# filevich/freeimpala

Measured on AMD Instinct MI355X. Metric: learner env-steps/sec (T×B/step) at T=100 B=4096, 1/2/4/8 MI355X, higher is better.
Workload: dtype bf16; 1 GPU; config#3 Atari-shaped conv policy 84x84x4, bf16 MFMA GEMMs + fp32 V-trace; T=100, B_per_gpu=4096, A=18, global_batch=4096, seq_len=100, parallelism=dp1, optimizer=adam, policy=atari

## Files before the change

freeimpala_amd/build_info.py:

```python
from __future__ import annotations

import glob
import hashlib
import os

ROOT = os.path.dirname(os.path.dirname(os.path.abspath(__file__)))


def source_files():
    files = sorted(glob.glob(os.path.join(ROOT, "freeimpala_amd", "csrc", "*")))
    files = [f for f in files if os.path.basename(f) != "farmer.hip"]
    files += [os.path.join(ROOT, p) for p in ("include/fi_learner.h", "Makefile")]
    return [f for f in files if os.path.isfile(f)]


def source_hash() -> str:
    h = hashlib.sha256()
    for f in source_files():
        h.update(os.path.relpath(f, ROOT).encode() + b"\0")
        with open(f, "rb") as fh:
            h.update(fh.read())
        h.update(b"\0")
    return h.hexdigest()[:16]


KERNEL_ENV = ("FI_FR_GRID", "FI_KEEP_DA1", "FI_BWD_UNFUSED", "FI_FWD_UNFUSED",
              "FI_A1_NHWC", "FI_ATARI_GENERIC")


def rocm_version() -> str:
    for p in ("/opt/rocm/.info/version", "/opt/rocm/.info/version-dev"):
        try:
            with open(p) as fh:
                return fh.read().strip()
        except OSError:
            pass
    return "unknown"


def runtime_key() -> dict:
    return {"env": {k: os.environ[k] for k in KERNEL_ENV if k in os.environ}, "rocm": rocm_version()}

# ... 11 lines not shown
```

freeimpala_amd/csrc/atari.h:

```cpp
#pragma once

#include <hip/hip_runtime.h>
#include <stdint.h>

#include <vector>

namespace fi {

constexpr int kC1Segs = 8;

struct KernelTagger {
    virtual void begin(const char* name) = 0;
    virtual void end() = 0;
    virtual ~KernelTagger() {}
};
struct TagScope {
    KernelTagger* t;
    TagScope(KernelTagger* t_, const char* name) : t(t_) {
        if (t) t->begin(name);
    }
    ~TagScope() {
        if (t) t->end();
    }
};
// ... 1 lines not shown
struct GradReadyHook {
    virtual int ready(size_t off, size_t n) = 0;
    virtual ~GradReadyHook() {}
};

struct AtariNet {
    static constexpr size_t kFrameBytes = 84 * 84 * 4;
    int B = 0, T = 0, A = 0, N = 0;
    void* impl = nullptr;
};

size_t atari_param_count(int A);
void atari_init_params(int A, uint64_t seed, std::vector<float>& p);
AtariNet* atari_create(int B, int T, int A);
void atari_destroy(AtariNet* n);
int atari_sync_weights(AtariNet* n, const float* params, hipStream_t s);
int atari_forward(AtariNet* n, const uint8_t* frames, float* logits, float* values, hipStream_t s,
                  KernelTagger* tg = nullptr);
int atari_backward(AtariNet* n, const uint8_t* frames, const float* dlogits, const float* dvalue,
                   float* grads, hipStream_t s, KernelTagger* tg = nullptr, GradReadyHook* gr = nullptr);
bool atari_tensor(AtariNet* n, const char* name, void** p, size_t* bytes);

}
```

freeimpala_amd/csrc/atari.hip:

```cpp
#include <algorithm>
#include <cstdlib>
#include <vector>

#include "atari.h"
#include "fi_common.h"
#include "kernels.h"

namespace fi {

typedef __bf16 bf16x8 __attribute__((ext_vector_type(8)));
typedef __bf16 bf16x4 __attribute__((ext_vector_type(4)));
typedef float f32x16 __attribute__((ext_vector_type(16)));
typedef unsigned int u32x4 __attribute__((ext_vector_type(4)));

namespace geo {
constexpr int C1K = 256, C1O = 32;
constexpr int C2K = 512, C2O = 64;
constexpr int C3K = 576, C3O = 64;
constexpr int FCK = 3136, FCO = 512;
constexpr int HP = 32;
constexpr int P1 = 400, P2 = 81, P3 = 49;
}

struct Offsets {
// ... 538 lines not shown
                              __bf16* dh, int R, int TB, float* fcb_slab, hipStream_t s) {
    FI_TRY(heads_dispatch(O, [&](auto o) {
        hipLaunchKernelGGL(heads_dgrad_valu<decltype(o)::value>, dim3(kHeadsDgradGrid), dim3(256), 0, s, dlog,
                           dval, wh, h, dh, R, TB, fcb_slab);
        return FI_OK;
    }));
    FI_HIP_CHECK(hipGetLastError());
    return FI_OK;
}

struct WeightsBf16 {
    __bf16 *c1T, *c2T, *c3T, *fcT, *hT;
    __bf16 *c2D, *c3D, *fcB;
};

__global__ void weights_bf16_kernel(const float* __restrict__ p, Offsets o, int A, WeightsBf16 w) {
    const int O = A + 1;
    const size_t n1 = 32 * 256, n2 = 64 * 512, n3 = 64 * 576, nf = (size_t)512 * 3136,
                 nh = 32 * 512, n2d = 4 * 32 * 256, n3d = 64 * 576, nfb = nf;
    const size_t total = n1 + n2 + n3 + nf + nh + n2d + n3d + nfb;
    for (size_t t = blockIdx.x * (size_t)blockDim.x + threadIdx.x; t < total;
         t += (size_t)gridDim.x * blockDim.x) {
        size_t i = t;
        if (i < n1) { const int co = i / 256, k = i % 256; w.c1T[i] = (__bf16)p[o.c1w + (size_t)k * 32 + co]; continue; }
        i -= n1;
        if (i < n2) { const int co = i / 512, k = i % 512; w.c2T[i] = (__bf16)p[o.c2w + (size_t)k * 64 + co]; continue; }
        i -= n2;
        if (i < n3) { const int co = i / 576, k = i % 576; w.c3T[i] = (__bf16)p[o.c3w + (size_t)k * 64 + co]; continue; }
        i -= n3;
        if (i < nf) { const size_t j = i / 3136, k = i % 3136; w.fcT[i] = (__bf16)p[o.fcw + k * 512 + j]; continue; }
        i -= nf;
        if (i < nh) { const int oo = i / 512, j = i % 512; w.hT[i] = (__bf16)(oo < O ? p[o.hw + (size_t)j * O + oo] : 0.f); continue; }
        i -= nh;
        if (i < n2d) {
            const int cls = i / (32 * 256), r = i % (32 * 256), ci = r / 256, k = r % 256;
// ... 18 lines not shown
    Offsets off{18};
    WeightsBf16 wb{};
    __bf16 *a1 = nullptr, *a2 = nullptr, *a3 = nullptr, *h = nullptr;
    __bf16 *da1 = nullptr, *da2 = nullptr, *da3 = nullptr, *dh = nullptr;
    float* slab = nullptr;
    size_t slab_floats = 0;
    const float* params = nullptr;
    std::vector<void*> allocs;
    int cs2 = 0, cs3 = 0;
    bool fr = true;
    bool fuse12 = true;
    bool fuse21 = true;
    bool keep_da1 = false;
    bool a1_planar = true;
    int fr_grid = 256;
};

int conv1_fwd_fr_launch(const uint8_t* frames, const __bf16* w1t, const float* bias, __bf16* a1,
                        int nframes, int grid, hipStream_t s);
int conv2_fwd_fr_launch(const __bf16* a1, const __bf16* w2t, const float* bias, __bf16* a2, int nframes,
                        int grid, hipStream_t s);
int conv3_fwd_fr_launch(const __bf16* a2, const __bf16* w3t, const float* bias, __bf16* a3, int nframes,
                        int grid, hipStream_t s);
int conv12_fwd_fr_launch(const uint8_t* frames, const __bf16* w1t, const float* b1, const __bf16* w2t,
                         const float* b2, __bf16* a1, __bf16* a2, int nframes, int grid, hipStream_t s,
                         int a1_planar);
int conv1_wgrad_fr_launch(const uint8_t* frames, const __bf16* da1, float* slab, float* cs_slab,
                          int nframes, int grid, hipStream_t s);
int conv21_bwd_fr_launch(const __bf16* a1, const __bf16* da2, const __bf16* w2d, const uint8_t* frames,
                         __bf16* da1_out, float* slab2, float* cs2, float* slab1, float* cs1, int nframes,
// ... 36 lines not shown
    I->a1_planar = I->fr && I->fuse12 && I->fuse21 && std::getenv("FI_A1_NHWC") == nullptr;
    if (const char* g = std::getenv("FI_FR_GRID")) I->fr_grid = std::max(1, std::min(256, std::atoi(g)));
    I->cs2 = (int)(((N * 100) + GBM - 1) / GBM * GBM);
    I->cs3 = (int)(((N * 81) + GBM - 1) / GBM * GBM);
    bool ok = dmalloc(I, &I->a1, N * 400 * 32) && dmalloc(I, &I->a2, N * 81 * 64) &&
              dmalloc(I, &I->a3, N * 3136) && dmalloc(I, &I->h, N * 512) &&
              dmalloc(I, &I->da1, N * 400 * 32) && dmalloc(I, &I->da2, N * 81 * 64) &&
              dmalloc(I, &I->da3, N * 3136) && dmalloc(I, &I->dh, N * 512) &&
              dmalloc(I, &I->wb.c1T, 32 * 256) && dmalloc(I, &I->wb.c2T, 64 * 512) &&
              dmalloc(I, &I->wb.c3T, 64 * 576) && dmalloc(I, &I->wb.fcT, (size_t)512 * 3136) &&
              dmalloc(I, &I->wb.hT, 32 * 512) && dmalloc(I, &I->wb.c2D, 4 * 32 * 256) &&
              dmalloc(I, &I->wb.c3D, 64 * 576) && dmalloc(I, &I->wb.fcB, (size_t)3136 * 512);
    const size_t s_fc = (size_t)SPL_FC * 3136 * 512, s_c3 = (size_t)SPL_C3 * 576 * 64,
                 s_c2 = (size_t)SPL_C2 * (512 * 64 + kC1Segs * 256 * 32), s_c1 = (size_t)SPL_C1 * 256 * 32,
                 s_h = (size_t)kHeadsGrid * 512 * 19;
    I->slab_floats = std::max(std::max(s_fc, s_c3), std::max(std::max(s_c2, s_c1), s_h)) + 1024 * 512;
    ok = ok && dmalloc(I, &I->slab, I->slab_floats);
    if (!ok) {
        set_error("atari: hipMalloc failed for activations");
        atari_destroy(n);
        return nullptr;
    }
    hipStream_t s0;
    if (hipStreamCreate(&s0) != hipSuccess) {
        set_error("atari: hipStreamCreate failed");
        atari_destroy(n);
        return nullptr;
    }
    if (hipMemsetAsync(I->dh, 0, N * 512 * sizeof(__bf16), s0) != hipSuccess ||
        hipMemsetAsync(I->da3, 0, N * 3136 * sizeof(__bf16), s0) != hipSuccess ||
        hipMemsetAsync(I->da2, 0, N * 81 * 64 * sizeof(__bf16), s0) != hipSuccess ||
        hipMemsetAsync(I->da1, 0, N * 400 * 32 * sizeof(__bf16), s0) != hipSuccess || hipStreamSynchronize(s0) != hipSuccess) {
// ... 4 lines not shown
    }
    (void)hipStreamDestroy(s0);
    return n;
}

void atari_destroy(AtariNet* n) {
    if (!n) return;
    AtariImpl* I = impl(n);
    if (I) {
        for (void* p : I->allocs) (void)hipFree(p);
        delete I;
    }
    delete n;
}

int atari_sync_weights(AtariNet* n, const float* params, hipStream_t s) {
    AtariImpl* I = impl(n);
    I->params = params;
    hipLaunchKernelGGL(weights_bf16_kernel, dim3(2048), dim3(256), 0, s, params, I->off, I->A, I->wb);
    FI_HIP_CHECK(hipGetLastError());
    return FI_OK;
}

int atari_forward(AtariNet* n, const uint8_t* frames, float* logits, float* values, hipStream_t s,
                  KernelTagger* tg) {
    AtariImpl* I = impl(n);
    const int N = I->N;
    const float* p = I->params;
    const Offsets& o = I->off;
    using namespace geo;
    int rc;
    if (I->fr && I->fuse12) {
        TagScope ts(tg, "conv12_fwd");
        rc = conv12_fwd_fr_launch(frames, I->wb.c1T, p + o.c1b, I->wb.c2T, p + o.c2b, I->a1, I->a2, N,
                                  std::min(N, I->fr_grid), s, I->a1_planar);
    } else if (I->fr) {
// ... 24 lines not shown
                             EpiHeadsOut{logits, values, p + o.hb, I->A}, N, HP, FCO, s); }
    return rc;
}

int atari_backward(AtariNet* n, const uint8_t* frames, const float* dlogits, const float* dvalue,
                   float* grads, hipStream_t s, KernelTagger* tg, GradReadyHook* gr) {
    AtariImpl* I = impl(n);
    const int N = I->N, A = I->A, O = A + 1;
    const int Nb = I->TB;
    const Offsets& o = I->off;
    using namespace geo;
    float* slab = I->slab;
    float* cs = I->slab + I->slab_floats - 1024 * 512;
    int rc;
#define FI_A(tag, x) do { TagScope ts_(tg, tag); rc = (x); if (rc) return rc; } while (0)
    FI_A("heads_wgrad", heads_wgrad_launch(O, dlogits, dvalue, I->h, slab, cs, Nb, I->TB, s));
    FI_A("reduce_slabs", reduce_slabs(slab, kHeadsGrid, (size_t)FCO * O, grads + o.hw, s));
    FI_A("reduce_slabs", reduce_slabs(cs, kHeadsGrid, (size_t)O, grads + o.hb, s));
    FI_A("heads_dgrad", heads_dgrad_launch(O, dlogits, dvalue, I->params + o.hw, I->h, I->dh, Nb, I->TB, slab, s));
    FI_A("reduce_slabs", reduce_slabs(slab, kHeadsDgradGrid, (size_t)FCO, grads + o.fcb, s));
    FI_A("fc_wgrad", fc_wgrad_launch(I->a3, I->dh, slab, grads + o.fcw, Nb, s));
    if (gr && (rc = gr->ready(o.fcw, o.total - o.fcw))) return rc;
    FI_A("fc_dgrad", fc_dgrad_launch(I->dh, I->wb.fcB, I->da3, I->fr ? Nb : N, s));
    if (I->fr) {
        const int grid = std::min(N, I->fr_grid);
        FI_A("conv3_bwd", conv3_bwd_fr_launch(I->a2, I->da3, I->a3, I->wb.c3D, I->da2, slab, cs, cs + (size_t)3 * grid * C2O,
                                              Nb, grid, s));
        FI_A("reduce_slabs", reduce_slabs(slab, grid, (size_t)C3K * C3O, grads + o.c3w, s));
        FI_A("reduce_slabs", reduce_slabs(cs, grid, (size_t)C3O, grads + o.c3b, s));
        if (gr && (rc = gr->ready(o.c3w, o.fcw - o.c3w))) return rc;
    } else {
        FI_A("relu_mask", relu_mask_bf16(I->da3, I->a3, (size_t)N * FCK, s));
        FI_A("conv3_wgrad", (wgrad<128, 64, 2, 2>(ConvGather<9, 64, 3, 1, 7>{I->a2, N * P3}, RowsBf16{I->da3, N * P3, C3O},
                                   slab, cs, N * P3, C3K, C3O, SPL_C3, 1.f, s)));
        FI_A("reduce_slabs", reduce_slabs(slab, SPL_C3, (size_t)C3K * C3O, grads + o.c3w, s));
        FI_A("reduce_slabs", reduce_slabs(cs, SPL_C3, (size_t)C3O, grads + o.c3b, s));
        FI_A("conv3_dgrad", (gemm<128, 64, 2, 2>(DgradGather<9, 3, 1, 7, 64>{I->da3, N, I->cs3},
                                  ClassRows{I->wb.c3D, 64, C3K, I->cs3, (size_t)64 * C3K, nullptr},
                                  EpiDgrad<9, 1>{I->da2, I->a2, N, I->cs3, 64}, I->cs3, 64, C3K, s)));
        if (gr && (rc = gr->ready(o.c3w, o.fcw - o.c3w))) return rc;
    }
    if (I->fr && I->fuse21) {
        const int grid = std::min(N, I->fr_grid);
        float* slab1 = slab + (size_t)grid * C2K * C2O;
        float* cs1 = cs + (size_t)grid * C2O;
        FI_A("conv21_bwd", conv21_bwd_fr_launch(I->a1, I->da2, I->wb.c2D, frames, I->keep_da1 ? I->da1 : nullptr,
                                                slab, cs + (size_t)3 * grid * C2O, slab1, cs1, Nb, grid, s, I->a1_planar));
        FI_A("reduce_slabs", reduce_slabs(slab, grid, (size_t)C2K * C2O, grads + o.c2w, s));
        FI_A("reduce_slabs", reduce_slabs(cs + (size_t)3 * grid * C2O, 2 * grid, (size_t)C2O, grads + o.c2b, s));
        FI_A("reduce_slabs", reduce_slabs(slab1, grid * kC1Segs, (size_t)C1K * C1O, grads + o.c1w, s));
        FI_A("reduce_slabs", reduce_slabs(cs1, 4 * grid, (size_t)C1O, grads + o.c1b, s));
        if (gr && (rc = gr->ready(0, o.c3w))) return rc;
        return FI_OK;
    }
    if (I->fr) {
        const int grid = std::min(N, I->fr_grid);
        FI_A("conv2_bwd", conv2_bwd_fr_launch(I->a1, I->da2, I->wb.c2D, I->da1, slab, cs + (size_t)3 * grid * C2O, Nb,
                                              grid, s));
        FI_A("reduce_slabs", reduce_slabs(slab, grid, (size_t)C2K * C2O, grads + o.c2w, s));
        FI_A("reduce_slabs", reduce_slabs(cs + (size_t)3 * grid * C2O, 2 * grid, (size_t)C2O, grads + o.c2b, s));
    } else {
        FI_A("conv2_wgrad", (wgrad<128, 64, 2, 2>(ConvGather<20, 32, 4, 2, 9>{I->a1, N * P2}, RowsBf16{I->da2, N * P2, C2O},
                               slab, cs, N * P2, C2K, C2O, SPL_C2, 1.f, s)));
        FI_A("reduce_slabs", reduce_slabs(slab, SPL_C2, (size_t)C2K * C2O, grads + o.c2w, s));
        FI_A("reduce_slabs", reduce_slabs(cs, SPL_C2, (size_t)C2O, grads + o.c2b, s));
        FI_A("conv2_dgrad", (gemm<128, 32, 4, 1>(DgradGather<20, 4, 2, 9, 64>{I->da2, N, I->cs2},
                              ClassRows{I->wb.c2D, 32, 256, I->cs2, (size_t)32 * 256, nullptr},
                              EpiDgrad<20, 2>{I->da1, I->a1, N, I->cs2, 32}, 4 * I->cs2, 32, 256, s)));
    }
    if (I->fr) {
        const int grid = std::min(N, I->fr_grid);
        FI_A("conv1_wgrad", conv1_wgrad_fr_launch(frames, I->da1, slab, cs, Nb, grid, s));
        FI_A("reduce_slabs", reduce_slabs(slab, grid, (size_t)C1K * C1O, grads + o.c1w, s));
        FI_A("reduce_slabs", reduce_slabs(cs, grid, (size_t)C1O, grads + o.c1b, s));
    } else {
        FI_A("conv1_wgrad", (wgrad<128, 32, 4, 1>(Conv1Gather{frames, N * P1}, RowsBf16{I->da1, N * P1, C1O}, slab, cs,
                                   N * P1, C1K, C1O, SPL_C1, 1.0f / 255.0f, s)));
        FI_A("reduce_slabs", reduce_slabs(slab, SPL_C1, (size_t)C1K * C1O, grads + o.c1w, s));
        FI_A("reduce_slabs", reduce_slabs(cs, SPL_C1, (size_t)C1O, grads + o.c1b, s));
    }
    if (gr && (rc = gr->ready(0, o.c3w))) return rc;
#undef FI_A
    return FI_OK;
}

bool atari_tensor(AtariNet* n, const char* name, void** p, size_t* bytes) {
    AtariImpl* I = impl(n);
    const size_t N = I->N;
    struct E {
        const char* nm;
        void* p;
        size_t b;
    } t[] = {{"a1", I->a1, N * 400 * 32 * 2}, {"a2", I->a2, N * 81 * 64 * 2},
             {"a3", I->a3, N * 3136 * 2},     {"h", I->h, N * 512 * 2},
             {"da1", I->da1, N * 400 * 32 * 2}, {"da2", I->da2, N * 81 * 64 * 2},
             {"da3", I->da3, N * 3136 * 2},   {"dh", I->dh, N * 512 * 2}};
// ... 11 lines not shown
```

freeimpala_amd/csrc/fc_gemm.hip:

```cpp
#include <algorithm>

#include "fi_common.h"
#include "kernels.h"

namespace fi {
namespace fcg {

typedef __bf16 bf16x8 __attribute__((ext_vector_type(8)));
typedef __bf16 bf16x4 __attribute__((ext_vector_type(4)));
typedef float f32x4 __attribute__((ext_vector_type(4)));
typedef int i32x2 __attribute__((ext_vector_type(2)));
typedef int i32x4 __attribute__((ext_vector_type(4)));
typedef __attribute__((address_space(3))) bf16x4 lds_bf16x4;

constexpr int FCK = 3136, FCO = 512;

__device__ __forceinline__ void dma16(fi_i32x4 rsrc, uint32_t voff, uint32_t lds_base) {
    uint32_t keep;
    asm volatile(
        "s_nop 4\n\t"
        "s_mov_b32 %0, m0\n\t"
        "s_mov_b32 m0, %3\n\t"
        "s_nop 0\n\t"
        "buffer_load_dwordx4 %1, %2, 0 offen lds\n\t"
// ... 498 lines not shown
}

int fc_wgrad_splits(int rows) {
    return std::max(1, std::min(9, (rows + 255) / 256));
}

template <int BX, int BY, int WX, int WY, int BK, int NS>
static int fc_wgrad_impl(const __bf16* a3, const __bf16* dh, float* slab, float* dw, int rows, hipStream_t s,
                         int S) {
    FI_REQUIRE(rows > 0, "fc_wgrad: rows must be positive");
    const int rps = ((rows + S - 1) / S + BK - 1) / BK * BK;
    const int nblk = S * (FCO / BX) * (FCK / BY);
    hipLaunchKernelGGL((fc_tn_kernel<BX, BY, WX, WY, BK, NS>), dim3(nblk), dim3(512), 0, s, dh, FCO, a3, FCK, rows, rps,
                       slab);
    FI_HIP_CHECK(hipGetLastError());
    return reduce_slabs(slab, S, (size_t)FCK * FCO, dw, s);
}

int fc_fwd_launch(const __bf16* a3, const __bf16* wT, const float* bias, __bf16* h, int rows, hipStream_t s) {
    return fc_fwd_impl<FC_FW_CFG>(a3, wT, bias, h, rows, s);
}
int fc_dgrad_launch(const __bf16* dh, const __bf16* w, __bf16* da3, int rows, hipStream_t s) {
    return fc_dgrad_impl<FC_DG_CFG>(dh, w, da3, rows, s);
}
int fc_wgrad_launch(const __bf16* a3, const __bf16* dh, float* slab, float* dw, int rows, hipStream_t s) {
    return fc_wgrad_impl<FC_WG_CFG>(a3, dh, slab, dw, rows, s, fc_wgrad_splits(rows));
}

}
```

freeimpala_amd/csrc/kernels.h:

```cpp
#pragma once

#include <hip/hip_runtime.h>
#include <stdint.h>

#include "fi_learner.h"

namespace fi {

struct HeadsGrad {
    const float* dlog;
    const float* dval;
    int rows;
    int TB;
    int A;
};

size_t vtrace_workspace_bytes(int T, int B, int A);
int vtrace_launch(int variant, int T, int B, int A, const float* pi, const float* mu,
                  const int32_t* act, const float* rew, const float* disc, const float* val,
                  const fi_vtrace_hparams& hp, float* vs, float* adv, float* dlog, float* dval,
                  double* losses, void* ws, size_t ws_bytes, hipStream_t stream,
                  bool finalize = true, int* nblk_out = nullptr, int* bad = nullptr);
int vtrace_finalize_launch(void* ws, int nblk, double* losses, hipStream_t stream,
                           const int* bad = nullptr);
// ... 17 lines not shown
                        float* cs_slab, int grid, hipStream_t s);

int colsum_partial(const float* Y, int M, int N, int splits, float* slab, hipStream_t s);
int heads_colsum_partial(const HeadsGrad& g, int splits, float* slab, hipStream_t s);
int f32_gemm_nt(const float* X, int ldx, int M, int K, const float* W, const float* bias, int N,
                bool relu, float* Y, hipStream_t s);
int f32_gemm_nn_dgrad(const float* dY, int M, int N, const float* W, int K, const float* act, float* dX,
                      hipStream_t s);
int f32_gemm_tn_wgrad(const float* dY, int M, int N, const float* X, int ldx, int K, int splits, float* slab,
                      hipStream_t s);
int fc_fwd_launch(const __bf16* a3, const __bf16* wT, const float* bias, __bf16* h, int rows, hipStream_t s);
int fc_dgrad_launch(const __bf16* dh, const __bf16* w, __bf16* da3, int rows, hipStream_t s);
int fc_wgrad_splits(int rows);
int fc_wgrad_launch(const __bf16* a3, const __bf16* dh, float* slab, float* dw, int rows, hipStream_t s);
int reduce_slabs(float* slab, int splits, size_t count, float* out, hipStream_t s);
int grad_sqnorm(const float* g, size_t n, double* part, int nblk, double* out, hipStream_t s,
                const double* vt_part = nullptr, int vt_nblk = 0, double* vt_losses = nullptr,
                int* nonfinite = nullptr);
int optimizer_step(int opt, float* p, const float* g, float* m, float* v, size_t n, float lr,
                   float b1, float b2, float eps, double bc1, double bc2, const double* sqnorm,
                   float max_norm, hipStream_t s, int* skip = nullptr);
int to_bf16(const float* src, uint16_t* dst, size_t n, hipStream_t s);
int fill_hash_bf16(void* dst, size_t n, uint32_t seed, hipStream_t s);
int synth_launch(uint64_t seed, int T, int B, int B_glob, int b_off, int A, int D, float gamma,
                 float* obs, float* mu, int32_t* act, float* rew, float* disc, uint8_t* frames,
                 hipStream_t s);
int ingest_launch(const void* rec, int T, int B, int A, int D, size_t entry_bytes, float* obs,
                  float* mu, int32_t* act, float* rew, float* disc, hipStream_t s, int* bad = nullptr);
int ingest_atari_launch(const void* rec, int T, int B, int A, size_t entry_bytes, uint8_t* frames,
                        float* mu, int32_t* act, float* rew, float* disc, hipStream_t s,
                        int* bad = nullptr);
int ingest_atari_planes_launch(const void* rec, int T, int B, int A, size_t entry_bytes, uint8_t* frames,
                               float* mu, int32_t* act, float* rew, float* disc, hipStream_t s,
                               int* bad = nullptr);

}
// ... 1 lines not shown
```

freeimpala_amd/csrc/learner.cpp:

```cpp
#include <hip/hip_runtime.h>
#include <rccl/rccl.h>

#include <algorithm>
#include <chrono>
#include <cstdio>
#include <cstdlib>
#include <cmath>
#include <cstring>
#include <new>
#include <string>
#include <thread>
#include <vector>

#include "atari.h"
#include "fi_common.h"
#include "kernels.h"

namespace fi {

static thread_local std::string g_err;
void set_error(const std::string& msg) { g_err = msg; }
int fail(int code, const std::string& msg) {
    g_err = msg;
    return code;
// ... 539 lines not shown
    }
    mark(l, FI_PHASE_BACKWARD);
    BucketAllReduce bar(l);
    if (l->cfg.arch == FI_ARCH_MLP) FI_TRY(mlp_backward(l, &bar));
    else {
        LearnerTagger tg(l);
        FI_TRY(atari_backward(l->atari, l->frames, l->dlogits, l->dvalue, l->grads, l->stream,
                              l->profiling ? &tg : nullptr, &bar));
    }
    mark(l, FI_PHASE_ALLREDUCE);
    {
        Tag t(l, "allreduce_wait");
        FI_TRY(bar.join());
    }
    mark(l, FI_PHASE_OPTIMIZER);
    {
        Tag t(l, "grad_norm");
        FI_TRY(grad_sqnorm(l->grads, l->nparams, l->small + 8, kSqParts, l->small + 3, l->stream,
                           vtrace_partials(l->vt_ws), vt_nblk, l->small, l->bad + 1));
    }
    const int step = l->step_count + 1;
    const double bc1 = 1.0 - std::pow((double)l->cfg.beta1, step);
    const double bc2 = 1.0 - std::pow((double)l->cfg.beta2, step);
    {
        Tag t(l, "optimizer");
        FI_TRY(optimizer_step(l->cfg.optimizer, l->params, l->grads, l->opt_m, l->opt_v, l->nparams,
                              l->cfg.lr, l->cfg.beta1, l->cfg.beta2, l->cfg.eps, bc1, bc2,
                              l->small + 3, l->cfg.max_grad_norm, l->stream, l->bad));
    }
    if (l->atari) {
        Tag t(l, "weights_bf16");
        FI_TRY(atari_sync_weights(l->atari, l->params, l->stream));
    }
    mark(l, FI_PHASE_COUNT);
    if (out) FI_HIP_CHECK(hipEventRecord(l->ev_b, l->stream));
    l->step_count = step;
    l->version++;
    if (sync) {
        FI_HIP_CHECK(hipStreamSynchronize(l->stream));
        if (l->profiling) {
            for (int p = 0; p < FI_PHASE_COUNT; ++p) {
                float ms = 0.f;
                FI_HIP_CHECK(hipEventElapsedTime(&ms, l->ev[p], l->ev[p + 1]));
                l->phase_sum[p] += ms;
            }
            l->phase_steps++;
            collect_tags(l);
// ... 512 lines not shown
```

freeimpala_amd/csrc/misc.hip:

```cpp
#include <algorithm>

#include "fi_common.h"
#include "kernels.h"

namespace fi {

__device__ __forceinline__ float approx_normal(uint4 u) {
    const uint32_t s = (u.x >> 8) + (u.y >> 8) + (u.z >> 8) + (u.w >> 8);
    const float x = (float)((int32_t)s - (int32_t)(1u << 25));
    return x * 0x1.bb67aep-24f;
}

__global__ void synth_normal_kernel(uint64_t seed, uint32_t stream, int rows, int B, int B_glob,
                                    int b_off, int D, float* out) {
    const size_t n = (size_t)rows * B * D;
    for (size_t i = blockIdx.x * (size_t)blockDim.x + threadIdx.x; i < n;
         i += (size_t)gridDim.x * blockDim.x) {
        const size_t lrow = i / D;
        const int d = (int)(i - lrow * D);
        const int t = (int)(lrow / B), b = (int)(lrow - (size_t)t * B);
        const uint64_t row = (uint64_t)t * B_glob + (uint64_t)(b_off + b);
        out[i] = approx_normal(philox4(seed, row * D + d, stream));
    }
}
// ... 349 lines not shown
int reduce_slabs(float* slab, int splits, size_t count, float* out, hipStream_t s) {
    if (splits >= 4 * kSlabGroup && count < 32768) {
        const int groups = (splits + kSlabGroup - 1) / kSlabGroup;
        hipLaunchKernelGGL(reduce_slabs_stage1, dim3((unsigned)((count + 63) / 64), (unsigned)groups), dim3(64), 0, s,
                           slab, splits, count);
        hipLaunchKernelGGL(reduce_slabs_kernel, dim3((unsigned)((count + 63) / 64)), dim3(256), 0, s, slab, groups,
                           count, (size_t)kSlabGroup * count, out);
    } else {
        hipLaunchKernelGGL(reduce_slabs_kernel, dim3((unsigned)((count + 63) / 64)), dim3(256), 0, s, slab, splits,
                           count, count, out);
    }
    FI_HIP_CHECK(hipGetLastError());
    return FI_OK;
}

__global__ void sqnorm_part_kernel(const float* __restrict__ g, size_t n, double* part) {
    __shared__ double red[4];
    double s = 0.0;
    for (size_t i = blockIdx.x * (size_t)blockDim.x + threadIdx.x; i < n;
         i += (size_t)gridDim.x * blockDim.x)
        s += (double)g[i] * (double)g[i];
    s = wave_sum(s);
    if ((threadIdx.x & 63) == 0) red[threadIdx.x >> 6] = s;
    __syncthreads();
    if (threadIdx.x == 0) part[blockIdx.x] = (red[0] + red[1]) + (red[2] + red[3]);
}

__global__ void sqnorm_final_kernel(const double* part, int nblk, double* out, const double* vt_part,
                                    int vt_nblk, double* vt_losses, int* nonfinite) {
    __shared__ double red[4][4];
// ... 14 lines not shown
        red[2][threadIdx.x >> 6] = l1;
        red[3][threadIdx.x >> 6] = l2;
    }
    __syncthreads();
    if (threadIdx.x < 4) {
        const double* r = red[threadIdx.x];
        const double v = (r[0] + r[1]) + (r[2] + r[3]);
        if (threadIdx.x == 0) {
            *out = v;
            if (nonfinite)
                *nonfinite = (__double_as_longlong(v) & 0x7FF0000000000000LL) == 0x7FF0000000000000LL;
        } else if (vt_losses) vt_losses[threadIdx.x - 1] = v;
    }
}

int grad_sqnorm(const float* g, size_t n, double* part, int nblk, double* out, hipStream_t s,
                const double* vt_part, int vt_nblk, double* vt_losses, int* nonfinite) {
    hipLaunchKernelGGL(sqnorm_part_kernel, dim3(nblk), dim3(256), 0, s, g, n, part);
    hipLaunchKernelGGL(sqnorm_final_kernel, dim3(1), dim3(256), 0, s, part, nblk, out, vt_part,
                       vt_losses ? vt_nblk : 0, vt_losses, nonfinite);
    FI_HIP_CHECK(hipGetLastError());
    return FI_OK;
}

__device__ __forceinline__ bool skip_update(int* skip) {
    if (!skip || (skip[0] | skip[1]) == 0) return false;
    if (blockIdx.x == 0 && threadIdx.x == 0) {
        skip[2] += 1;
        skip[3] |= (skip[0] != 0 ? 1 : 0) | (skip[1] != 0 ? 2 : 0);
    }
    return true;
}

__global__ void adam_kernel(float* __restrict__ p, const float* __restrict__ g,
                            float* __restrict__ m, float* __restrict__ v, size_t n, float lr,
                            float b1, float b2, float eps, double bc1, double bc2,
                            const double* sqnorm, float max_norm, int* skip) {
    if (skip_update(skip)) return;
    float scale = 1.f;
    if (max_norm > 0.f) {
        const double norm = sqrt(*sqnorm);
        if (norm > max_norm) scale = (float)((double)max_norm / (norm + 1e-6));
    }
    for (size_t i = blockIdx.x * (size_t)blockDim.x + threadIdx.x; i < n;
         i += (size_t)gridDim.x * blockDim.x) {
        const float gi = g[i] * scale;
        const float mi = b1 * m[i] + (1.0f - b1) * gi;
        const float vi = b2 * v[i] + (1.0f - b2) * gi * gi;
        m[i] = mi;
        v[i] = vi;
        const double mh = mi / bc1, vh = vi / bc2;
        p[i] = (float)(p[i] - lr * mh / (sqrt(vh) + eps));
    }
}

__global__ void sgd_kernel(float* __restrict__ p, const float* __restrict__ g, size_t n, float lr,
                           const double* sqnorm, float max_norm, int* skip) {
    if (skip_update(skip)) return;
    float scale = 1.f;
    if (max_norm > 0.f) {
        const double norm = sqrt(*sqnorm);
        if (norm > max_norm) scale = (float)((double)max_norm / (norm + 1e-6));
    }
    for (size_t i = blockIdx.x * (size_t)blockDim.x + threadIdx.x; i < n;
         i += (size_t)gridDim.x * blockDim.x)
        p[i] -= lr * (g[i] * scale);
}

int optimizer_step(int opt, float* p, const float* g, float* m, float* v, size_t n, float lr,
                   float b1, float b2, float eps, double bc1, double bc2, const double* sqnorm,
                   float max_norm, hipStream_t s, int* skip) {
    if (opt == FI_OPT_ADAM)
        hipLaunchKernelGGL(adam_kernel, dim3(grid_for(n)), dim3(256), 0, s, p, g, m, v, n, lr, b1,
                           b2, eps, bc1, bc2, sqnorm, max_norm, skip);
    else
        hipLaunchKernelGGL(sgd_kernel, dim3(grid_for(n)), dim3(256), 0, s, p, g, n, lr, sqnorm,
                           max_norm, skip);
    FI_HIP_CHECK(hipGetLastError());
    return FI_OK;
}

// ... 64 lines not shown
```

Baseline: 16.84 million env-steps/s.

## Batch slab reductions per backward stage and fuse norm finalize into optimizer

Replaces the many per-tensor slab reductions in the Atari backward with one segmented reduction launch per stage, driven by a device-side segment table. The fc weight-gradient slab moves to its own offset so it can be reduced together with the heads and fc-bias slabs. The grad-norm finalize step is folded into a fused optimizer tail kernel, which also writes the bf16 fc weight image directly, so weights_bf16 skips that section. This cuts kernel launches and one pass over the large fc weight, but makes the slab layout more complex and increases slab memory.

```diff
diff --git a/freeimpala_amd/build_info.py b/freeimpala_amd/build_info.py
--- a/freeimpala_amd/build_info.py
+++ b/freeimpala_amd/build_info.py
@@ -25,7 +25,7 @@
 
 
 KERNEL_ENV = ("FI_FR_GRID", "FI_KEEP_DA1", "FI_BWD_UNFUSED", "FI_FWD_UNFUSED",
-              "FI_A1_NHWC", "FI_ATARI_GENERIC")
+              "FI_A1_NHWC", "FI_ATARI_GENERIC", "FI_SLAB_PER_TENSOR")
 
 
 def rocm_version() -> str:
diff --git a/freeimpala_amd/csrc/atari.h b/freeimpala_amd/csrc/atari.h
--- a/freeimpala_amd/csrc/atari.h
+++ b/freeimpala_amd/csrc/atari.h
@@ -39,7 +39,9 @@
 void atari_init_params(int A, uint64_t seed, std::vector<float>& p);
 AtariNet* atari_create(int B, int T, int A);
 void atari_destroy(AtariNet* n);
-int atari_sync_weights(AtariNet* n, const float* params, hipStream_t s);
+int atari_sync_weights(AtariNet* n, const float* params, hipStream_t s, bool fcb_done = false);
+bool atari_bucket_reduce(AtariNet* n);
+void atari_fcb_image(AtariNet* n, uint16_t** img, size_t* off, size_t* count);
 int atari_forward(AtariNet* n, const uint8_t* frames, float* logits, float* values, hipStream_t s,
                   KernelTagger* tg = nullptr);
 int atari_backward(AtariNet* n, const uint8_t* frames, const float* dlogits, const float* dvalue,
diff --git a/freeimpala_amd/csrc/atari.hip b/freeimpala_amd/csrc/atari.hip
--- a/freeimpala_amd/csrc/atari.hip
+++ b/freeimpala_amd/csrc/atari.hip
@@ -576,11 +576,11 @@
     __bf16 *c2D, *c3D, *fcB;
 };
 
-__global__ void weights_bf16_kernel(const float* __restrict__ p, Offsets o, int A, WeightsBf16 w) {
+__global__ void weights_bf16_kernel(const float* __restrict__ p, Offsets o, int A, WeightsBf16 w, int with_fcB) {
     const int O = A + 1;
     const size_t n1 = 32 * 256, n2 = 64 * 512, n3 = 64 * 576, nf = (size_t)512 * 3136,
                  nh = 32 * 512, n2d = 4 * 32 * 256, n3d = 64 * 576, nfb = nf;
-    const size_t total = n1 + n2 + n3 + nf + nh + n2d + n3d + nfb;
+    const size_t total = n1 + n2 + n3 + nf + nh + n2d + n3d + (with_fcB ? nfb : 0);
     for (size_t t = blockIdx.x * (size_t)blockDim.x + threadIdx.x; t < total;
          t += (size_t)gridDim.x * blockDim.x) {
         size_t i = t;
@@ -629,6 +629,10 @@
     bool keep_da1 = false;
     bool a1_planar = true;
     int fr_grid = 256;
+    bool seg_reduce = false;
+    SlabSeg* segs = nullptr;
+    int seg_first[3] = {}, seg_n[3] = {}, seg_blocks[3] = {};
+    size_t fcb_slab = 0, fcw_slab = 0;
 };
 
 int conv1_fwd_fr_launch(const uint8_t* frames, const __bf16* w1t, const float* bias, __bf16* a1,
@@ -695,8 +699,39 @@
     const size_t s_fc = (size_t)SPL_FC * 3136 * 512, s_c3 = (size_t)SPL_C3 * 576 * 64,
                  s_c2 = (size_t)SPL_C2 * (512 * 64 + kC1Segs * 256 * 32), s_c1 = (size_t)SPL_C1 * 256 * 32,
                  s_h = (size_t)kHeadsGrid * 512 * 19;
-    I->slab_floats = std::max(std::max(s_fc, s_c3), std::max(std::max(s_c2, s_c1), s_h)) + 1024 * 512;
+    const size_t s_fcb = (size_t)kHeadsDgradGrid * 512;
+    I->seg_reduce = I->fr && I->fuse21 && std::getenv("FI_SLAB_PER_TENSOR") == nullptr;
+    const size_t s_b0 = I->seg_reduce ? s_h + s_fcb + s_fc : 0;
+    I->slab_floats = std::max(std::max(std::max(s_fc, s_c3), s_b0), std::max(std::max(s_c2, s_c1), s_h)) + 1024 * 512;
     ok = ok && dmalloc(I, &I->slab, I->slab_floats);
+    if (ok && I->seg_reduce) {
+        using namespace geo;
+        I->fcb_slab = s_h;
+        I->fcw_slab = s_h + s_fcb;
+        const Offsets& o = I->off;
+        const int O = A + 1, grid = (int)std::min<size_t>(N, (size_t)I->fr_grid);
+        const size_t cs = I->slab_floats - 1024 * 512;
+        SlabSeg t[10] = {
+            {0, o.hw, kHeadsGrid, FCO * O},
+            {cs, o.hb, kHeadsGrid, O},
+            {I->fcb_slab, o.fcb, kHeadsDgradGrid, FCO},
+            {I->fcw_slab, o.fcw, fc_wgrad_splits(I->TB), FCK * FCO},
+            {0, o.c3w, grid, C3K * C3O},
+            {cs, o.c3b, grid, C3O},
+            {0, o.c2w, grid, C2K * C2O},
+            {cs + (size_t)3 * grid * C2O, o.c2b, 2 * grid, C2O},
+            {(size_t)grid * C2K * C2O, o.c1w, grid * kC1Segs, C1K * C1O},
+            {cs + (size_t)grid * C2O, o.c1b, 4 * grid, C1O},
+        };
+        const int first[3] = {0, 4, 6}, cnt[3] = {4, 2, 4};
+        for (int b = 0; b < 3; ++b) {
+            I->seg_first[b] = first[b];
+            I->seg_n[b] = cnt[b];
+            I->seg_blocks[b] = slab_segments_plan(t + first[b], cnt[b]);
+            ok = ok && I->seg_blocks[b] > 0;
+        }
+        ok = ok && dmalloc(I, &I->segs, 10) && hipMemcpy(I->segs, t, sizeof(t), hipMemcpyHostToDevice) == hipSuccess;
+    }
     if (!ok) {
         set_error("atari: hipMalloc failed for activations");
         atari_destroy(n);
@@ -731,12 +766,22 @@
     delete n;
 }
 
-int atari_sync_weights(AtariNet* n, const float* params, hipStream_t s) {
+int atari_sync_weights(AtariNet* n, const float* params, hipStream_t s, bool fcb_done) {
     AtariImpl* I = impl(n);
     I->params = params;
-    hipLaunchKernelGGL(weights_bf16_kernel, dim3(2048), dim3(256), 0, s, params, I->off, I->A, I->wb);
+    hipLaunchKernelGGL(weights_bf16_kernel, dim3(fcb_done ? 1024 : 2048), dim3(256), 0, s, params, I->off, I->A, I->wb,
+                       fcb_done ? 0 : 1);
     FI_HIP_CHECK(hipGetLastError());
     return FI_OK;
+}
+
+bool atari_bucket_reduce(AtariNet* n) { return impl(n)->seg_reduce; }
+
+void atari_fcb_image(AtariNet* n, uint16_t** img, size_t* off, size_t* count) {
+    AtariImpl* I = impl(n);
+    *img = (uint16_t*)I->wb.fcB;
+    *off = I->off.fcw;
+    *count = (size_t)3136 * 512;
 }
 
 int atari_forward(AtariNet* n, const uint8_t* frames, float* logits, float* values, hipStream_t s,
@@ -791,20 +836,30 @@
     float* cs = I->slab + I->slab_floats - 1024 * 512;
     int rc;
 #define FI_A(tag, x) do { TagScope ts_(tg, tag); rc = (x); if (rc) return rc; } while (0)
+    const bool seg = I->seg_reduce;
+#define FI_SEG(b) FI_A("reduce_slabs", reduce_segments(I->segs + I->seg_first[b], I->seg_n[b], I->seg_blocks[b], slab, \
+                                                        grads, s))
     FI_A("heads_wgrad", heads_wgrad_launch(O, dlogits, dvalue, I->h, slab, cs, Nb, I->TB, s));
-    FI_A("reduce_slabs", reduce_slabs(slab, kHeadsGrid, (size_t)FCO * O, grads + o.hw, s));
-    FI_A("reduce_slabs", reduce_slabs(cs, kHeadsGrid, (size_t)O, grads + o.hb, s));
-    FI_A("heads_dgrad", heads_dgrad_launch(O, dlogits, dvalue, I->params + o.hw, I->h, I->dh, Nb, I->TB, slab, s));
-    FI_A("reduce_slabs", reduce_slabs(slab, kHeadsDgradGrid, (size_t)FCO, grads + o.fcb, s));
-    FI_A("fc_wgrad", fc_wgrad_launch(I->a3, I->dh, slab, grads + o.fcw, Nb, s));
+    if (!seg) {
+        FI_A("reduce_slabs", reduce_slabs(slab, kHeadsGrid, (size_t)FCO * O, grads + o.hw, s));
+        FI_A("reduce_slabs", reduce_slabs(cs, kHeadsGrid, (size_t)O, grads + o.hb, s));
+    }
+    FI_A("heads_dgrad", heads_dgrad_launch(O, dlogits, dvalue, I->params + o.hw, I->h, I->dh, Nb, I->TB,
+                                           slab + I->fcb_slab, s));
+    if (!seg) FI_A("reduce_slabs", reduce_slabs(slab, kHeadsDgradGrid, (size_t)FCO, grads + o.fcb, s));
+    FI_A("fc_wgrad", fc_wgrad_launch(I->a3, I->dh, slab + I->fcw_slab, seg ? nullptr : grads + o.fcw, Nb, s));
+    if (seg) FI_SEG(0);
     if (gr && (rc = gr->ready(o.fcw, o.total - o.fcw))) return rc;
     FI_A("fc_dgrad", fc_dgrad_launch(I->dh, I->wb.fcB, I->da3, I->fr ? Nb : N, s));
     if (I->fr) {
         const int grid = std::min(N, I->fr_grid);
         FI_A("conv3_bwd", conv3_bwd_fr_launch(I->a2, I->da3, I->a3, I->wb.c3D, I->da2, slab, cs, cs + (size_t)3 * grid * C2O,
                                               Nb, grid, s));
-        FI_A("reduce_slabs", reduce_slabs(slab, grid, (size_t)C3K * C3O, grads + o.c3w, s));
-        FI_A("reduce_slabs", reduce_slabs(cs, grid, (size_t)C3O, grads + o.c3b, s));
+        if (seg) FI_SEG(1);
+        else {
+            FI_A("reduce_slabs", reduce_slabs(slab, grid, (size_t)C3K * C3O, grads + o.c3w, s));
+            FI_A("reduce_slabs", reduce_slabs(cs, grid, (size_t)C3O, grads + o.c3b, s));
+        }
         if (gr && (rc = gr->ready(o.c3w, o.fcw - o.c3w))) return rc;
     } else {
         FI_A("relu_mask", relu_mask_bf16(I->da3, I->a3, (size_t)N * FCK, s));
@@ -823,10 +878,13 @@
         float* cs1 = cs + (size_t)grid * C2O;
         FI_A("conv21_bwd", conv21_bwd_fr_launch(I->a1, I->da2, I->wb.c2D, frames, I->keep_da1 ? I->da1 : nullptr,
                                                 slab, cs + (size_t)3 * grid * C2O, slab1, cs1, Nb, grid, s, I->a1_planar));
-        FI_A("reduce_slabs", reduce_slabs(slab, grid, (size_t)C2K * C2O, grads + o.c2w, s));
-        FI_A("reduce_slabs", reduce_slabs(cs + (size_t)3 * grid * C2O, 2 * grid, (size_t)C2O, grads + o.c2b, s));
-        FI_A("reduce_slabs", reduce_slabs(slab1, grid * kC1Segs, (size_t)C1K * C1O, grads + o.c1w, s));
-        FI_A("reduce_slabs", reduce_slabs(cs1, 4 * grid, (size_t)C1O, grads + o.c1b, s));
+        if (seg) FI_SEG(2);
+        else {
+            FI_A("reduce_slabs", reduce_slabs(slab, grid, (size_t)C2K * C2O, grads + o.c2w, s));
+            FI_A("reduce_slabs", reduce_slabs(cs + (size_t)3 * grid * C2O, 2 * grid, (size_t)C2O, grads + o.c2b, s));
+            FI_A("reduce_slabs", reduce_slabs(slab1, grid * kC1Segs, (size_t)C1K * C1O, grads + o.c1w, s));
+            FI_A("reduce_slabs", reduce_slabs(cs1, 4 * grid, (size_t)C1O, grads + o.c1b, s));
+        }
         if (gr && (rc = gr->ready(0, o.c3w))) return rc;
         return FI_OK;
     }
@@ -857,6 +915,7 @@
         FI_A("reduce_slabs", reduce_slabs(cs, SPL_C1, (size_t)C1O, grads + o.c1b, s));
     }
     if (gr && (rc = gr->ready(0, o.c3w))) return rc;
+#undef FI_SEG
 #undef FI_A
     return FI_OK;
 }
diff --git a/freeimpala_amd/csrc/fc_gemm.hip b/freeimpala_amd/csrc/fc_gemm.hip
--- a/freeimpala_amd/csrc/fc_gemm.hip
+++ b/freeimpala_amd/csrc/fc_gemm.hip
@@ -536,6 +536,7 @@
     hipLaunchKernelGGL((fc_tn_kernel<BX, BY, WX, WY, BK, NS>), dim3(nblk), dim3(512), 0, s, dh, FCO, a3, FCK, rows, rps,
                        slab);
     FI_HIP_CHECK(hipGetLastError());
+    if (!dw) return FI_OK;
     return reduce_slabs(slab, S, (size_t)FCK * FCO, dw, s);
 }
 
diff --git a/freeimpala_amd/csrc/kernels.h b/freeimpala_amd/csrc/kernels.h
--- a/freeimpala_amd/csrc/kernels.h
+++ b/freeimpala_amd/csrc/kernels.h
@@ -55,12 +55,25 @@
 int fc_wgrad_splits(int rows);
 int fc_wgrad_launch(const __bf16* a3, const __bf16* dh, float* slab, float* dw, int rows, hipStream_t s);
 int reduce_slabs(float* slab, int splits, size_t count, float* out, hipStream_t s);
+struct SlabSeg {
+    unsigned long long slab_off, out_off;
+    int splits, count;
+    int groups;
+    int blk0;
+};
+int slab_segments_plan(SlabSeg* segs, int n);
+int reduce_segments(const SlabSeg* segs, int n, int blocks, const float* slab, float* out, hipStream_t s);
 int grad_sqnorm(const float* g, size_t n, double* part, int nblk, double* out, hipStream_t s,
                 const double* vt_part = nullptr, int vt_nblk = 0, double* vt_losses = nullptr,
                 int* nonfinite = nullptr);
 int optimizer_step(int opt, float* p, const float* g, float* m, float* v, size_t n, float lr,
                    float b1, float b2, float eps, double bc1, double bc2, const double* sqnorm,
                    float max_norm, hipStream_t s, int* skip = nullptr);
+int grad_sqnorm_partials(const float* g, size_t n, double* part, int nblk, hipStream_t s);
+int optimizer_tail_step(int opt, float* p, const float* g, float* m, float* v, size_t n, float lr, float b1,
+                        float b2, float eps, double bc1, double bc2, float max_norm, hipStream_t s, int* skip,
+                        const double* part, int nblk, double* sqnorm, const double* vt_part, int vt_nblk,
+                        double* vt_losses, uint16_t* img, size_t img_off, size_t img_n);
 int to_bf16(const float* src, uint16_t* dst, size_t n, hipStream_t s);
 int fill_hash_bf16(void* dst, size_t n, uint32_t seed, hipStream_t s);
 int synth_launch(uint64_t seed, int T, int B, int B_glob, int b_off, int A, int D, float gamma,
diff --git a/freeimpala_amd/csrc/learner.cpp b/freeimpala_amd/csrc/learner.cpp
--- a/freeimpala_amd/csrc/learner.cpp
+++ b/freeimpala_amd/csrc/learner.cpp
@@ -577,23 +577,42 @@
         FI_TRY(bar.join());
     }
     mark(l, FI_PHASE_OPTIMIZER);
-    {
-        Tag t(l, "grad_norm");
-        FI_TRY(grad_sqnorm(l->grads, l->nparams, l->small + 8, kSqParts, l->small + 3, l->stream,
-                           vtrace_partials(l->vt_ws), vt_nblk, l->small, l->bad + 1));
-    }
     const int step = l->step_count + 1;
     const double bc1 = 1.0 - std::pow((double)l->cfg.beta1, step);
     const double bc2 = 1.0 - std::pow((double)l->cfg.beta2, step);
-    {
-        Tag t(l, "optimizer");
-        FI_TRY(optimizer_step(l->cfg.optimizer, l->params, l->grads, l->opt_m, l->opt_v, l->nparams,
-                              l->cfg.lr, l->cfg.beta1, l->cfg.beta2, l->cfg.eps, bc1, bc2,
-                              l->small + 3, l->cfg.max_grad_norm, l->stream, l->bad));
-    }
-    if (l->atari) {
+    if (l->atari && atari_bucket_reduce(l->atari)) {
+        {
+            Tag t(l, "grad_norm");
+            FI_TRY(grad_sqnorm_partials(l->grads, l->nparams, l->small + 8, kSqParts, l->stream));
+        }
+        uint16_t* img;
+        size_t img_off, img_n;
+        atari_fcb_image(l->atari, &img, &img_off, &img_n);
+        {
+            Tag t(l, "optimizer");
+            FI_TRY(optimizer_tail_step(l->cfg.optimizer, l->params, l->grads, l->opt_m, l->opt_v, l->nparams,
+                                       l->cfg.lr, l->cfg.beta1, l->cfg.beta2, l->cfg.eps, bc1, bc2,
+                                       l->cfg.max_grad_norm, l->stream, l->bad, l->small + 8, kSqParts, l->small + 3,
+                                       vtrace_partials(l->vt_ws), vt_nblk, l->small, img, img_off, img_n));
+        }
         Tag t(l, "weights_bf16");
-        FI_TRY(atari_sync_weights(l->atari, l->params, l->stream));
+        FI_TRY(atari_sync_weights(l->atari, l->params, l->stream, true));
+    } else {
+        {
+            Tag t(l, "grad_norm");
+            FI_TRY(grad_sqnorm(l->grads, l->nparams, l->small + 8, kSqParts, l->small + 3, l->stream,
+                               vtrace_partials(l->vt_ws), vt_nblk, l->small, l->bad + 1));
+        }
+        {
+            Tag t(l, "optimizer");
+            FI_TRY(optimizer_step(l->cfg.optimizer, l->params, l->grads, l->opt_m, l->opt_v, l->nparams,
+                                  l->cfg.lr, l->cfg.beta1, l->cfg.beta2, l->cfg.eps, bc1, bc2,
+                                  l->small + 3, l->cfg.max_grad_norm, l->stream, l->bad));
+        }
+        if (l->atari) {
+            Tag t(l, "weights_bf16");
+            FI_TRY(atari_sync_weights(l->atari, l->params, l->stream));
+        }
     }
     mark(l, FI_PHASE_COUNT);
     if (out) FI_HIP_CHECK(hipEventRecord(l->ev_b, l->stream));
diff --git a/freeimpala_amd/csrc/misc.hip b/freeimpala_amd/csrc/misc.hip
--- a/freeimpala_amd/csrc/misc.hip
+++ b/freeimpala_amd/csrc/misc.hip
@@ -387,6 +387,109 @@
     return FI_OK;
 }
 
+__device__ __forceinline__ float slab_role_sum(const float* p, int terms, size_t stride, int w) {
+    float a0 = 0.f, a1 = 0.f, a2 = 0.f, a3 = 0.f;
+    int k = w;
+#pragma unroll 4
+    for (; k + 12 < terms; k += 16) {
+        a0 += p[(size_t)k * stride];
+        a1 += p[(size_t)(k + 4) * stride];
+        a2 += p[(size_t)(k + 8) * stride];
+        a3 += p[(size_t)(k + 12) * stride];
+    }
+    for (; k < terms; k += 4) a0 += p[(size_t)k * stride];
+    return (a0 + a1) + (a2 + a3);
+}
+
+__device__ __forceinline__ float slab_group_sum(const float* p, int k0, int k1, size_t count) {
+    float a0 = 0.f, a1 = 0.f, a2 = 0.f, a3 = 0.f;
+    if (k1 - k0 == kSlabGroup) {
+        float v[kSlabGroup];
+#pragma unroll
+        for (int j = 0; j < kSlabGroup; ++j) v[j] = p[(size_t)(k0 + j) * count];
+#pragma unroll
+        for (int j = 0; j < kSlabGroup; j += 4) {
+            a0 += v[j];
+            a1 += v[j + 1];
+            a2 += v[j + 2];
+            a3 += v[j + 3];
+        }
+    } else {
+        int k = k0;
+        for (; k + 3 < k1; k += 4) {
+            a0 += p[(size_t)k * count];
+            a1 += p[(size_t)(k + 1) * count];
+            a2 += p[(size_t)(k + 2) * count];
+            a3 += p[(size_t)(k + 3) * count];
+        }
+        for (; k < k1; ++k) a0 += p[(size_t)k * count];
+    }
+    return (a0 + a1) + (a2 + a3);
+}
+
+constexpr int kSegThreads = 1024, kSegMaxGroups = 64, kSlabSerial = 16;
+__global__ __launch_bounds__(kSegThreads) void reduce_segments_kernel(const SlabSeg* __restrict__ segs, int nseg,
+                                                                      const float* __restrict__ slab_base,
+                                                                      float* __restrict__ out_base) {
+    __shared__ float part[kSegMaxGroups][64];
+    __shared__ float red[16][64];
+    int sg = 0;
+    while (sg + 1 < nseg && (int)blockIdx.x >= segs[sg + 1].blk0) ++sg;
+    const SlabSeg g = segs[sg];
+    const int b = (int)blockIdx.x - g.blk0;
+    const int lane = threadIdx.x & 63, wv = threadIdx.x >> 6;
+    const float* slab = slab_base + g.slab_off;
+    float* out = out_base + g.out_off;
+    const size_t count = (size_t)g.count;
+    if (g.groups > 0) {
+        const size_t i = (size_t)b * 64 + lane;
+        for (int grp = wv; grp < g.groups; grp += kSegThreads / 64) {
+            const int k0 = grp * kSlabGroup;
+            part[grp][lane] = i < count ? slab_group_sum(slab + i, k0, min(g.splits, k0 + kSlabGroup), count) : 0.f;
+        }
+        __syncthreads();
+        if (wv < 4) red[wv][lane] = slab_role_sum(&part[0][lane], g.groups, 64, wv);
+        __syncthreads();
+        if (wv == 0 && i < count) out[i] = (red[0][lane] + red[1][lane]) + (red[2][lane] + red[3][lane]);
+    } else if (g.splits <= kSlabSerial) {
+        const size_t i = (size_t)b * kSegThreads + threadIdx.x;
+        if (i < count) {
+            const float r0 = slab_role_sum(slab + i, g.splits, count, 0), r1 = slab_role_sum(slab + i, g.splits, count, 1),
+                        r2 = slab_role_sum(slab + i, g.splits, count, 2), r3 = slab_role_sum(slab + i, g.splits, count, 3);
+            out[i] = (r0 + r1) + (r2 + r3);
+        }
+    } else {
+        const int w = wv & 3;
+        const size_t i = ((size_t)b * 4 + (wv >> 2)) * 64 + lane;
+        red[wv][lane] = i < count ? slab_role_sum(slab + i, g.splits, count, w) : 0.f;
+        __syncthreads();
+        const int t = wv & ~3;
+        if (w == 0 && i < count) out[i] = (red[t][lane] + red[t + 1][lane]) + (red[t + 2][lane] + red[t + 3][lane]);
+    }
+}
+
+int slab_segments_plan(SlabSeg* segs, int n) {
+    int blk = 0;
+    for (int j = 0; j < n; ++j) {
+        SlabSeg& g = segs[j];
+        if (g.splits < 1 || g.count < 1) return -1;
+        const int xtiles = (g.count + 63) / 64;
+        const bool narrow = g.splits >= 4 * kSlabGroup && g.count < 32768;
+        g.groups = narrow ? (g.splits + kSlabGroup - 1) / kSlabGroup : 0;
+        if (g.groups > kSegMaxGroups) return -1;
+        g.blk0 = blk;
+        blk += narrow ? xtiles : g.splits <= kSlabSerial ? (g.count + kSegThreads - 1) / kSegThreads : (xtiles + 3) / 4;
+    }
+    return blk;
+}
+
+int reduce_segments(const SlabSeg* segs, int n, int blocks, const float* slab, float* out, hipStream_t s) {
+    FI_REQUIRE(segs && n >= 1 && blocks >= 1 && slab && out, "reduce_segments: bad argument");
+    hipLaunchKernelGGL(reduce_segments_kernel, dim3((unsigned)blocks), dim3(kSegThreads), 0, s, segs, n, slab, out);
+    FI_HIP_CHECK(hipGetLastError());
+    return FI_OK;
+}
+
 __global__ void sqnorm_part_kernel(const float* __restrict__ g, size_t n, double* part) {
     __shared__ double red[4];
     double s = 0.0;
@@ -431,6 +534,12 @@
     }
 }
 
+int grad_sqnorm_partials(const float* g, size_t n, double* part, int nblk, hipStream_t s) {
+    hipLaunchKernelGGL(sqnorm_part_kernel, dim3(nblk), dim3(256), 0, s, g, n, part);
+    FI_HIP_CHECK(hipGetLastError());
+    return FI_OK;
+}
+
 int grad_sqnorm(const float* g, size_t n, double* part, int nblk, double* out, hipStream_t s,
                 const double* vt_part, int vt_nblk, double* vt_losses, int* nonfinite) {
     hipLaunchKernelGGL(sqnorm_part_kernel, dim3(nblk), dim3(256), 0, s, g, n, part);
@@ -447,6 +556,28 @@
         skip[3] |= (skip[0] != 0 ? 1 : 0) | (skip[1] != 0 ? 2 : 0);
     }
     return true;
+}
+
+__device__ __forceinline__ float adam_update(float* __restrict__ p, const float* __restrict__ g,
+                                             float* __restrict__ m, float* __restrict__ v, size_t i, float scale,
+                                             float lr, float b1, float b2, float eps, double bc1, double bc2) {
+#pragma clang fp contract(off)
+    const float gi = g[i] * scale;
+    const float mi = b1 * m[i] + (1.0f - b1) * gi;
+    const float vi = b2 * v[i] + (1.0f - b2) * gi * gi;
+    m[i] = mi;
+    v[i] = vi;
+    const double mh = mi / bc1, vh = vi / bc2;
+    const float pn = (float)(p[i] - lr * mh / (sqrt(vh) + eps));
+    p[i] = pn;
+    return pn;
+}
+
+__device__ __forceinline__ float sgd_update(float* __restrict__ p, const float* __restrict__ g, size_t i, float scale,
+                                            float lr) {
+    const float pn = __builtin_fmaf(-lr, g[i] * scale, p[i]);
+    p[i] = pn;
+    return pn;
 }
 
 __global__ void adam_kernel(float* __restrict__ p, const float* __restrict__ g,
@@ -460,15 +591,8 @@
         if (norm > max_norm) scale = (float)((double)max_norm / (norm + 1e-6));
     }
     for (size_t i = blockIdx.x * (size_t)blockDim.x + threadIdx.x; i < n;
-         i += (size_t)gridDim.x * blockDim.x) {
-        const float gi = g[i] * scale;
-        const float mi = b1 * m[i] + (1.0f - b1) * gi;
-        const float vi = b2 * v[i] + (1.0f - b2) * gi * gi;
-        m[i] = mi;
-        v[i] = vi;
-        const double mh = mi / bc1, vh = vi / bc2;
-        p[i] = (float)(p[i] - lr * mh / (sqrt(vh) + eps));
-    }
+         i += (size_t)gridDim.x * blockDim.x)
+        adam_update(p, g, m, v, i, scale, lr, b1, b2, eps, bc1, bc2);
 }
 
 __global__ void sgd_kernel(float* __restrict__ p, const float* __restrict__ g, size_t n, float lr,
@@ -481,7 +605,98 @@
     }
     for (size_t i = blockIdx.x * (size_t)blockDim.x + threadIdx.x; i < n;
          i += (size_t)gridDim.x * blockDim.x)
-        p[i] -= lr * (g[i] * scale);
+        sgd_update(p, g, i, scale, lr);
+}
+
+struct OptTail {
+    const double* part;
+    int nblk;
+    double* sqnorm;
+    const double* vt_part;
+    int vt_nblk;
+    double* vt_losses;
+    uint16_t* img;
+    size_t img_off, img_n;
+};
+
+template <bool ADAM>
+__global__ __launch_bounds__(256) void optimizer_tail_kernel(float* __restrict__ p, const float* __restrict__ g,
+                                                             float* __restrict__ m, float* __restrict__ v, size_t n,
+                                                             float lr, float b1, float b2, float eps, double bc1,
+                                                             double bc2, float max_norm, int* skip, OptTail t) {
+    __shared__ double red[4][4];
+    const bool lead = blockIdx.x == 0;
+    double s = 0.0, l0 = 0.0, l1 = 0.0, l2 = 0.0;
+    for (int i = threadIdx.x; i < t.nblk; i += blockDim.x) s += t.part[i];
+    s = wave_sum(s);
+    if (lead) {
+        for (int i = threadIdx.x; i < t.vt_nblk; i += blockDim.x) {
+            l0 += t.vt_part[(size_t)i * 3];
+            l1 += t.vt_part[(size_t)i * 3 + 1];
+            l2 += t.vt_part[(size_t)i * 3 + 2];
+        }
+        l0 = wave_sum(l0);
+        l1 = wave_sum(l1);
+        l2 = wave_sum(l2);
+    }
+    if ((threadIdx.x & 63) == 0) {
+        red[0][threadIdx.x >> 6] = s;
+        red[1][threadIdx.x >> 6] = l0;
+        red[2][threadIdx.x >> 6] = l1;
+        red[3][threadIdx.x >> 6] = l2;
+    }
+    __syncthreads();
+    const double sq = (red[0][0] + red[0][1]) + (red[0][2] + red[0][3]);
+    const bool nonfinite = (__double_as_longlong(sq) & 0x7FF0000000000000LL) == 0x7FF0000000000000LL;
+    const int bad_actions = skip[0];
+    if (lead && threadIdx.x < 4) {
+        if (threadIdx.x == 0) {
+            *t.sqnorm = sq;
+            skip[1] = nonfinite;
+        } else if (t.vt_losses) {
+            const double* r = red[threadIdx.x];
+            t.vt_losses[threadIdx.x - 1] = (r[0] + r[1]) + (r[2] + r[3]);
+        }
+    }
+    if (bad_actions != 0 || nonfinite) {
+        if (lead && threadIdx.x == 0) {
+            skip[2] += 1;
+            skip[3] |= (bad_actions != 0 ? 1 : 0) | (nonfinite ? 2 : 0);
+        }
+        return;
+    }
+    float scale = 1.f;
+    if (max_norm > 0.f) {
+        const double norm = sqrt(sq);
+        if (norm > max_norm) scale = (float)((double)max_norm / (norm + 1e-6));
+    }
+    for (size_t i = blockIdx.x * (size_t)blockDim.x + threadIdx.x; i < n;
+         i += (size_t)gridDim.x * blockDim.x) {
+        float pn;
+        if constexpr (ADAM) pn = adam_update(p, g, m, v, i, scale, lr, b1, b2, eps, bc1, bc2);
+        else pn = sgd_update(p, g, i, scale, lr);
+        if (t.img && i - t.img_off < t.img_n)
+            t.img[i - t.img_off] = __builtin_bit_cast(uint16_t, (__bf16)pn);
+    }
+}
+
+constexpr int kOptTailMaxGrid = 2048;
+
+int optimizer_tail_step(int opt, float* p, const float* g, float* m, float* v, size_t n, float lr, float b1,
+                        float b2, float eps, double bc1, double bc2, float max_norm, hipStream_t s, int* skip,
+                        const double* part, int nblk, double* sqnorm, const double* vt_part, int vt_nblk,
+                        double* vt_losses, uint16_t* img, size_t img_off, size_t img_n) {
+    FI_REQUIRE(skip && part && sqnorm && nblk >= 1, "optimizer_tail_step: bad argument");
+    const OptTail t{part, nblk, sqnorm, vt_part, vt_losses ? vt_nblk : 0, vt_losses, img, img_off, img_n};
+    const int grid = std::min(grid_for(n), kOptTailMaxGrid);
+    if (opt == FI_OPT_ADAM)
+        hipLaunchKernelGGL(optimizer_tail_kernel<true>, dim3(grid), dim3(256), 0, s, p, g, m, v, n, lr, b1, b2, eps,
+                           bc1, bc2, max_norm, skip, t);
+    else
+        hipLaunchKernelGGL(optimizer_tail_kernel<false>, dim3(grid), dim3(256), 0, s, p, g, m, v, n, lr, b1, b2,
+                           eps, bc1, bc2, max_norm, skip, t);
+    FI_HIP_CHECK(hipGetLastError());
+    return FI_OK;
 }
 
 int optimizer_step(int opt, float* p, const float* g, float* m, float* v, size_t n, float lr,
```

Measured after the change: 16.86 million env-steps/s, median of 6. About the same (+0.1%).
